# 2646207530/hamer-yolo

Measured on AMD Instinct MI355X. Metric: hands/sec (HaMeR ViT-H/16 + decoder + MANO forward; detector bypassed), higher is better.
Workload: dtype fp16; 1 GPU; BASELINE configs[1]: batch=64 synthetic 256x256 crops per GPU, HaMeR ViT-H/16 + 6-layer decoder + MANO, 16-bit MFMA (fp16 operands), crops resident in HBM; batch_per_gpu=64, global_batch=64, batches_in_flight=2, weights=seeded random-init fp32 master weights, rounded to the operand type at load, parallelism=crop-shard x1

## Files before the change

hamer_yolo_amd/csrc/attention.hip:

```cpp
#include "common.h"
#include "hamer_hip_internal.h"

namespace {

constexpr int T = 192;
constexpr int HD = 80;
constexpr int KSTR = 88;
constexpr int VSTR = 80;
constexpr int KS_BYTES = T * KSTR * 2;
constexpr int VT_BYTES = T * VSTR * 2;
constexpr int BUF_BYTES = KS_BYTES + VT_BYTES;
constexpr int NWAVE = T / 16;
constexpr int OTILE_BYTES = 16 * HD * 2;
constexpr int ATT_LDS = 2 * BUF_BYTES + NWAVE * OTILE_BYTES;
constexpr int ATT_LDS_TOME = ATT_LDS + 2 * T * 4;

template <class V4> __device__ __forceinline__ V4 lds_read_tr4(const void* p) {
  typedef __attribute__((ext_vector_type(4))) short s16x4;
  const s16x4 v = __builtin_amdgcn_ds_read_tr16_b64_v4i16((__attribute__((address_space(3))) s16x4*)p);
  return __builtin_bit_cast(V4, v);
}

__device__ __forceinline__ void glds16_hidden(const void* gsrc, void* lds_wave_base) {
  const unsigned dst = __builtin_amdgcn_readfirstlane((unsigned)(uintptr_t)(__attribute__((address_space(3))) void*)lds_wave_base);
  asm volatile("s_mov_b32 m0, %1\n\ts_nop 0\n\tglobal_load_lds_dwordx4 %0, off" :: "v"(gsrc), "s"(dst) : "memory");
}

__device__ __forceinline__ void wait_vm0() {
  __builtin_amdgcn_s_waitcnt(0x0F70);
  asm volatile("" ::: "memory");
}

constexpr int HDP = 96;
typedef __attribute__((ext_vector_type(4))) int v4i_att;

template <class TT, bool MX8 = false, bool TOME = false>
__global__ __launch_bounds__(64 * NWAVE, 3) void vit_attention_kernel(const typename TT::elem* __restrict__ qkv,
                                                                    typename TT::elem* __restrict__ out, int heads,
                                                                    int items, float scale_log2e,
                                                                    unsigned char* __restrict__ out_scales = nullptr,
                                                                    const float* __restrict__ size = nullptr, int Tn = T) {
  extern __shared__ __attribute__((aligned(16))) char smem[];
  using elem = typename TT::elem;
  using vec8 = typename TT::vec8;
  using vec4 = typename TT::vec4;

  const int tid = threadIdx.x, lane = tid & 63;
  const int wave = __builtin_amdgcn_readfirstlane(tid >> 6);
  const int C = heads * HD;
  const size_t ld = (size_t)3 * C;
  const int g = lane >> 4, li = lane & 15;
  const int Tt = TOME ? Tn : T;
  vec8 zero8;
#pragma unroll
  for (int i = 0; i < 8; ++i) zero8[i] = (elem)0.0f;
  if constexpr (TOME) {
    for (int buf = 0; buf < 2; ++buf) {
      char* Vb = smem + buf * BUF_BYTES + KS_BYTES;
      for (int c = Tt * (VSTR / 8) + tid; c < T * (VSTR / 8); c += 64 * NWAVE) *(vec8*)(Vb + c * 16) = zero8;
    }
  }

  auto issue = [&](int item, int buf, vec8 (&qf)[3], float& szl) {
    const elem* base = qkv + (size_t)(item / heads) * Tt * ld + (size_t)(item % heads) * HD;
    char* Kb = smem + buf * BUF_BYTES;
    char* Vb = Kb + KS_BYTES;
    constexpr int KCH = T * (KSTR / 8), VCH = T * (VSTR / 8);
    const int kch = Tt * (KSTR / 8), vch = Tt * (VSTR / 8);
    for (int c0 = wave * 64; c0 < KCH; c0 += 64 * NWAVE) {
      const int c = c0 + lane, ch = c % (KSTR / 8);
      int t = c / (KSTR / 8);
      if (TOME) t = t < Tt ? t : Tt - 1;
      if (!TOME || c0 < kch) glds16_hidden(base + (size_t)t * ld + C + (ch < HD / 8 ? ch : 0) * 8, Kb + c0 * 16);
    }
    for (int c0 = wave * 64; c0 < VCH; c0 += 64 * NWAVE) {
      const int c = c0 + lane, ch = c % (VSTR / 8);
      int t = c / (VSTR / 8);
      if (TOME) t = t < Tt ? t : Tt - 1;
      if (!TOME || c0 < vch) glds16_hidden(base + (size_t)t * ld + 2 * C + ch * 8, Vb + c0 * 16);
    }
    const int qr = wave * 16 + li;
    const elem* qrow = base + (size_t)(TOME ? (qr < Tt ? qr : Tt - 1) : qr) * ld;
    if constexpr (TOME) szl = (size != nullptr && tid < Tt) ? size[(size_t)(item / heads) * Tt + tid] : 1.0f;
    qf[0] = *(const vec8*)(qrow + 8 * g);
    qf[1] = *(const vec8*)(qrow + 32 + 8 * g);
    qf[2] = g < 2 ? *(const vec8*)(qrow + 64 + 8 * g) : zero8;
  };

  auto compute = [&](int item, int buf, const vec8 (&qf)[3]) {
    const elem* Ks = (const elem*)(smem + buf * BUF_BYTES);
    const elem* Vs = (const elem*)(smem + buf * BUF_BYTES + KS_BYTES);
    const int b = item / heads, h = item % heads;
    const int q = wave * 16 + li;
    if constexpr (TOME) { if (wave * 16 >= Tt) return; }
    f32x4_t st[12];
    vec8 kf[2][2][3];
    auto load_k = [&](int kb, int pair) {
#pragma unroll
      for (int j = 0; j < 2; ++j) {
        const elem* krow = Ks + ((pair * 2 + j) * 16 + li) * KSTR + 8 * g;
        kf[kb][j][0] = *(const vec8*)(krow);
        kf[kb][j][1] = *(const vec8*)(krow + 32);
        kf[kb][j][2] = g < 2 ? *(const vec8*)(krow + 64) : zero8;
      }
    };
    load_k(0, 0);
#pragma unroll
    for (int pair = 0; pair < 6; ++pair) {
      if (pair + 1 < 6) load_k((pair + 1) & 1, pair + 1);
#pragma unroll
      for (int j = 0; j < 2; ++j) {
        f32x4_t acc = f32x4_t{0.f, 0.f, 0.f, 0.f};
        acc = TT::mfma(kf[pair & 1][j][0], qf[0], acc);
        acc = TT::mfma(kf[pair & 1][j][1], qf[1], acc);
        acc = TT::mfma(kf[pair & 1][j][2], qf[2], acc);
        st[pair * 2 + j] = acc;
      }
    }
    if constexpr (TOME) {
#pragma unroll
      for (int kt = 0; kt < 12; ++kt) {
        const f32x4_t lz = *(const f32x4_t*)(smem + ATT_LDS + (buf * T + kt * 16 + 4 * g) * 4);
#pragma unroll
        for (int r = 0; r < 4; ++r) st[kt][r] = (kt * 16 + 4 * g + r < Tt) ? fmaf(st[kt][r], scale_log2e, lz[r]) : -INFINITY;
      }
    }
    float m = st[0][0];
#pragma unroll
    for (int kt = 0; kt < 12; ++kt)
#pragma unroll
      for (int r = 0; r < 4; ++r) m = fmaxf(m, st[kt][r]);
    m = fmaxf(m, __shfl_xor(m, 16, 64));
    m = fmaxf(m, __shfl_xor(m, 32, 64));
    const float mneg = TOME ? -m : -m * scale_log2e;
    float sum4[4] = {0.f, 0.f, 0.f, 0.f};
#pragma unroll
    for (int kt = 0; kt < 12; ++kt)
#pragma unroll
      for (int r = 0; r < 4; ++r) {
        const float p = __builtin_amdgcn_exp2f(TOME ? st[kt][r] + (mneg + 14.0f) : fmaf(st[kt][r], scale_log2e, mneg));
        st[kt][r] = p;
        sum4[r] += p;
      }
    float sum = (sum4[0] + sum4[1]) + (sum4[2] + sum4[3]);
    sum += __shfl_xor(sum, 16, 64);
    sum += __shfl_xor(sum, 32, 64);
    const float inv = 1.0f / sum;

    vec8 pf[6], pl[TOME ? 6 : 1];
#pragma unroll
    for (int kk = 0; kk < 6; ++kk)
#pragma unroll
      for (int r = 0; r < 4; ++r) {
        pf[kk][r] = (elem)st[2 * kk][r];
        pf[kk][4 + r] = (elem)st[2 * kk + 1][r];
        if constexpr (TOME) {
          pl[kk][r] = (elem)(st[2 * kk][r] - (float)pf[kk][r]);
          pl[kk][4 + r] = (elem)(st[2 * kk + 1][r] - (float)pf[kk][4 + r]);
        }
      }

    const elem* vblk = Vs + (4 * g + (li >> 2)) * VSTR + 4 * (li & 3);
    vec4 vlo[2][5], vhi[2][5];
    auto load_v = [&](int vb, int kk) {
#pragma unroll
      for (int dt = 0; dt < 5; ++dt) {
        vlo[vb][dt] = lds_read_tr4<vec4>(vblk + (32 * kk) * VSTR + dt * 16);
        vhi[vb][dt] = lds_read_tr4<vec4>(vblk + (32 * kk + 16) * VSTR + dt * 16);
      }
    };
    f32x4_t oacc[5];
#pragma unroll
    for (int dt = 0; dt < 5; ++dt) oacc[dt] = f32x4_t{0.f, 0.f, 0.f, 0.f};
    if constexpr (!TOME) load_v(0, 0);
#pragma unroll
    for (int kk = 0; kk < 6; ++kk) {
      if constexpr (TOME) load_v(kk & 1, kk);
      else if (kk + 1 < 6) load_v((kk + 1) & 1, kk + 1);
#pragma unroll
      for (int dt = 0; dt < 5; ++dt) {
        vec8 vf;
#pragma unroll
        for (int i = 0; i < 4; ++i) { vf[i] = vlo[kk & 1][dt][i]; vf[4 + i] = vhi[kk & 1][dt][i]; }
        oacc[dt] = TT::mfma(vf, pf[kk], oacc[dt]);
        if constexpr (TOME) oacc[dt] = TT::mfma(vf, pl[kk], oacc[dt]);
      }
    }
    if constexpr (MX8) {
      const int Mrows = (items / heads) * T;
      float am[3] = {0.f, 0.f, 0.f};
#pragma unroll
      for (int dt = 0; dt < 5; ++dt)
#pragma unroll
        for (int r = 0; r < 4; ++r) am[dt >> 1] = fmaxf(am[dt >> 1], fabsf(oacc[dt][r] * inv));
      unsigned sb[3];
      float isc[3];
#pragma unroll
      for (int bk = 0; bk < 3; ++bk) {
        float a = am[bk];
        a = fmaxf(a, __shfl_xor(a, 16, 64));
        a = fmaxf(a, __shfl_xor(a, 32, 64));
        sb[bk] = mx8_scale_byte(a);
        isc[bk] = mx8_inv_scale(sb[bk]);
      }
      char* ot8 = smem + 2 * BUF_BYTES + wave * OTILE_BYTES;
#pragma unroll
      for (int dt = 0; dt < 6; ++dt) {
        int p = 0;
        if (dt < 5) {
          const float sc = inv * isc[dt >> 1];
          p = mx8_pack4(oacc[dt][0] * sc, oacc[dt][1] * sc, oacc[dt][2] * sc, oacc[dt][3] * sc);
        }
        *(int*)(ot8 + li * HDP + dt * 16 + 4 * g) = p;
      }
      char* obase8 = (char*)out + ((size_t)b * T + wave * 16) * (heads * HDP) + h * HDP;
#pragma unroll
      for (int c0 = 0; c0 < 16 * (HDP / 16); c0 += 64) {
        const int c = c0 + lane;
        if (c < 16 * (HDP / 16)) {
          const int row = c / (HDP / 16), ch = c % (HDP / 16);
          *(v4i_att*)(obase8 + (size_t)row * (heads * HDP) + ch * 16) = *(const v4i_att*)(ot8 + row * HDP + ch * 16);
        }
      }
      if (g == 0) {
#pragma unroll
        for (int bk = 0; bk < 3; ++bk) out_scales[(size_t)(h * 3 + bk) * Mrows + (size_t)b * T + q] = (unsigned char)sb[bk];
      }
      return;
    }
    elem* ot = (elem*)(smem + 2 * BUF_BYTES + wave * OTILE_BYTES);
#pragma unroll
    for (int dt = 0; dt < 5; ++dt) {
      vec4 o;
#pragma unroll
      for (int r = 0; r < 4; ++r) o[r] = (elem)(oacc[dt][r] * inv);
      *(vec4*)(ot + li * HD + dt * 16 + 4 * g) = o;
    }
    elem* obase = out + ((size_t)b * Tt + wave * 16) * C + h * HD;
#pragma unroll
    for (int c0 = 0; c0 < 16 * (HD / 8); c0 += 64) {
      const int c = c0 + lane;
      if (c < 16 * (HD / 8)) {
        const int row = c / (HD / 8), ch = c % (HD / 8);
        if (!TOME || wave * 16 + row < Tt) *(vec8*)(obase + (size_t)row * C + ch * 8) = *(const vec8*)(ot + row * HD + ch * 8);
      }
    }
  };

  vec8 qa[3], qb[3];
  float sza = 1.0f, szb = 1.0f;
  auto publish_size = [&](int buf, float szl) {
    if constexpr (TOME) { if (tid < Tt) *(float*)(smem + ATT_LDS + (buf * T + tid) * 4) = __builtin_amdgcn_logf(szl); }
  };
  int item = xcd_remap(blockIdx.x, gridDim.x);
  if (item < items) issue(item, 0, qa, sza);
  while (item < items) {
    wait_vm0();
    publish_size(0, sza);
    __builtin_amdgcn_s_barrier();
    int nxt = item + gridDim.x;
    if (nxt < items) issue(nxt, 1, qb, szb);
    compute(item, 0, qa);
    item = nxt;
    if (item >= items) break;
    wait_vm0();
    publish_size(1, szb);
    __builtin_amdgcn_s_barrier();
    nxt = item + gridDim.x;
    if (nxt < items) issue(nxt, 0, qa, sza);
    compute(item, 1, qb);
    item = nxt;
  }
}

int att_grid_for(int items, int n_cu) {
  if (const int v = hm_option(HM_OPT_ATT_GRID)) n_cu = v;
  const int per = (items + n_cu - 1) / n_cu;
  return (items + per - 1) / per;
}

template <class TT, bool MX8 = false, bool TOME = false>
int launch_att(const void* qkv, void* out, int B, int heads, float scale, hipStream_t s, void* out_scales = nullptr,
               const float* size = nullptr, int Tn = T) {
  static HmLdsOnce lds_once;
  auto kern = vit_attention_kernel<TT, MX8, TOME>;
  constexpr int LDS = TOME ? ATT_LDS_TOME : ATT_LDS;
  if (const int rc = lds_once.ensure((const void*)kern, LDS, "hm_vit_attention: cannot raise dynamic LDS limit")) return rc;
  const int n_cu = hm_device_cu_count();
  if (n_cu <= 0) return hm_set_error(HM_ERR_HIP, "hm_vit_attention: cannot query the device");
  const int items = B * heads;
  const int grid = att_grid_for(items, n_cu);
  hipLaunchKernelGGL(kern, dim3(grid), dim3(64 * NWAVE), LDS, s, (const typename TT::elem*)qkv,
                     (typename TT::elem*)out, heads, items, scale * 1.44269504088896340736f, (unsigned char*)out_scales, size, Tn);
  return hm_check_launch("hm_vit_attention");
}

}

extern "C" int hm_attention_grid(int items, int cus) {
  if (items <= 0) return 0;
  return att_grid_for(items, cus > 0 ? cus : 256);
}

int hm_attention_tome_launch(const void* qkv, const float* size, void* out, int B, int tokens, int heads, float scale, int dtype,
                             hipStream_t s) {
  if (tokens < 1 || tokens > T) return hm_set_error(HM_ERR_ARG, "hm_tome_attention: 0 < tokens <= 192");
  if (dtype == HM_DTYPE_BF16) return launch_att<TBf16, false, true>(qkv, out, B, heads, scale, s, nullptr, size, tokens);
  if (dtype == HM_DTYPE_F16) return launch_att<TF16, false, true>(qkv, out, B, heads, scale, s, nullptr, size, tokens);
  return hm_set_error(HM_ERR_ARG, "hm_tome_attention: bad dtype");
}

extern "C" int hm_vit_attention(const void* qkv, void* out, int B, int tokens, int heads, int head_dim, float scale,
                                int dtype, void* stream_) {
  hipStream_t s = (hipStream_t)stream_;
  if (!qkv || !out || B <= 0 || heads <= 0) return hm_set_error(HM_ERR_ARG, "hm_vit_attention: bad arguments");
  if (tokens != T || head_dim != HD)
    return hm_set_error(HM_ERR_ARG, "hm_vit_attention: built for 192 tokens and head_dim 80 (ViT-H/16 on 256x192)");
  if (((uintptr_t)qkv | (uintptr_t)out) & 15) return hm_set_error(HM_ERR_ARG, "hm_vit_attention: 16-byte alignment");
  HmProfScope prof(HM_K_ATTENTION, 0, B, heads, head_dim, s);
  if (dtype == HM_DTYPE_BF16) return launch_att<TBf16>(qkv, out, B, heads, scale, s);
  if (dtype == HM_DTYPE_F16) return launch_att<TF16>(qkv, out, B, heads, scale, s);
  return hm_set_error(HM_ERR_ARG, "hm_vit_attention: bad dtype");
}

extern "C" int hm_vit_attention_mx8(const void* qkv, void* out8, void* out_scales, int B, int tokens, int heads, int head_dim,
                                    float scale, void* stream_) {
  hipStream_t s = (hipStream_t)stream_;
  if (!qkv || !out8 || !out_scales || B <= 0 || heads <= 0) return hm_set_error(HM_ERR_ARG, "hm_vit_attention_mx8: bad arguments");
  if (tokens != T || head_dim != HD)
    return hm_set_error(HM_ERR_ARG, "hm_vit_attention_mx8: built for 192 tokens and head_dim 80 (ViT-H/16 on 256x192)");
  if (((uintptr_t)qkv | (uintptr_t)out8 | (uintptr_t)out_scales) & 15) return hm_set_error(HM_ERR_ARG, "hm_vit_attention_mx8: 16-byte alignment");
  HmProfScope prof(HM_K_ATTENTION, 1, B, heads, head_dim, s);
  return launch_att<TBf16, true>(qkv, out8, B, heads, scale, s, out_scales);
}
```

Baseline: 3728 hands/s.

## Use partial vmcnt waits and unconditional Q loads in attention prefetch ring

For the non-ToMe attention path, the kernel now waits only until the previous item's K/V loads retire (vmcnt<=3), leaving the next item's output stores in flight, instead of draining all outstanding memory ops each iteration. The third Q fragment is loaded without a lane-dependent branch, and the zero masking is moved into compute. Output write-back loops are flattened into fixed-count stores without bounds checks. The intent is to cut stalls from full vmcnt drains and from divergent tails. The risk is that the vmcnt count depends on the exact instruction ordering the compiler emits, which could cause correctness hazards.

Result: no change. 3730 hands/s (median of 2 runs) (+0.1%).

```diff
diff --git a/hamer_yolo_amd/csrc/attention.hip b/hamer_yolo_amd/csrc/attention.hip
--- a/hamer_yolo_amd/csrc/attention.hip
+++ b/hamer_yolo_amd/csrc/attention.hip
@@ -21,18 +21,20 @@
   return __builtin_bit_cast(V4, v);
 }
 
-__device__ __forceinline__ void glds16_hidden(const void* gsrc, void* lds_wave_base) {
-  const unsigned dst = __builtin_amdgcn_readfirstlane((unsigned)(uintptr_t)(__attribute__((address_space(3))) void*)lds_wave_base);
+__device__ __forceinline__ void glds16_hidden(const void* gsrc, unsigned lds_wave_base) {
+  const unsigned dst = __builtin_amdgcn_readfirstlane(lds_wave_base);
   asm volatile("s_mov_b32 m0, %1\n\ts_nop 0\n\tglobal_load_lds_dwordx4 %0, off" :: "v"(gsrc), "s"(dst) : "memory");
 }
 
-__device__ __forceinline__ void wait_vm0() {
-  __builtin_amdgcn_s_waitcnt(0x0F70);
+template <int N> __device__ __forceinline__ void wait_vm() {
+  static_assert(N >= 0 && N < 16, "vmcnt immediate");
   asm volatile("" ::: "memory");
-}
-
+  __builtin_amdgcn_s_waitcnt(0x0F70 | N);
+  asm volatile("" ::: "memory");
+}
 constexpr int HDP = 96;
 typedef __attribute__((ext_vector_type(4))) int v4i_att;
+typedef __attribute__((ext_vector_type(2))) int v2i_att;
 
 template <class TT, bool MX8 = false, bool TOME = false>
 __global__ __launch_bounds__(64 * NWAVE, 3) void vit_attention_kernel(const typename TT::elem* __restrict__ qkv,
@@ -51,6 +53,8 @@
   const size_t ld = (size_t)3 * C;
   const int g = lane >> 4, li = lane & 15;
   const int Tt = TOME ? Tn : T;
+  constexpr bool RING = !TOME;
+  constexpr int N_ST = 3;
   vec8 zero8;
 #pragma unroll
   for (int i = 0; i < 8; ++i) zero8[i] = (elem)0.0f;
@@ -61,11 +65,11 @@
     }
   }
 
-  auto issue = [&](int item, int buf, vec8 (&qf)[3], float& szl) {
-    const elem* base = qkv + (size_t)(item / heads) * Tt * ld + (size_t)(item % heads) * HD;
-    char* Kb = smem + buf * BUF_BYTES;
-    char* Vb = Kb + KS_BYTES;
-    constexpr int KCH = T * (KSTR / 8), VCH = T * (VSTR / 8);
+  constexpr int KCH_ALL = T * (KSTR / 8), VCH_ALL = T * (VSTR / 8);
+  auto copy_kv = [&](const elem* base, int buf) {
+    const unsigned Kb = (unsigned)(uintptr_t)(__attribute__((address_space(3))) char*)smem + buf * BUF_BYTES;
+    const unsigned Vb = Kb + KS_BYTES;
+    constexpr int KCH = KCH_ALL, VCH = VCH_ALL;
     const int kch = Tt * (KSTR / 8), vch = Tt * (VSTR / 8);
     for (int c0 = wave * 64; c0 < KCH; c0 += 64 * NWAVE) {
       const int c = c0 + lane, ch = c % (KSTR / 8);
@@ -79,12 +83,17 @@
       if (TOME) t = t < Tt ? t : Tt - 1;
       if (!TOME || c0 < vch) glds16_hidden(base + (size_t)t * ld + 2 * C + ch * 8, Vb + c0 * 16);
     }
+  };
+  auto issue = [&](int item, int buf, vec8 (&qf)[3], float& szl) {
+    const elem* base = qkv + (size_t)(item / heads) * Tt * ld + (size_t)(item % heads) * HD;
+    copy_kv(base, buf);
     const int qr = wave * 16 + li;
     const elem* qrow = base + (size_t)(TOME ? (qr < Tt ? qr : Tt - 1) : qr) * ld;
     if constexpr (TOME) szl = (size != nullptr && tid < Tt) ? size[(size_t)(item / heads) * Tt + tid] : 1.0f;
     qf[0] = *(const vec8*)(qrow + 8 * g);
     qf[1] = *(const vec8*)(qrow + 32 + 8 * g);
-    qf[2] = g < 2 ? *(const vec8*)(qrow + 64 + 8 * g) : zero8;
+    if constexpr (RING) qf[2] = *(const vec8*)(qrow + 64 + 8 * (g & 1));
+    else qf[2] = g < 2 ? *(const vec8*)(qrow + 64 + 8 * g) : zero8;
   };
 
   auto compute = [&](int item, int buf, const vec8 (&qf)[3]) {
@@ -95,6 +104,7 @@
     if constexpr (TOME) { if (wave * 16 >= Tt) return; }
     f32x4_t st[12];
     vec8 kf[2][2][3];
+    const vec8 q2 = (!RING || g < 2) ? qf[2] : zero8;
     auto load_k = [&](int kb, int pair) {
 #pragma unroll
       for (int j = 0; j < 2; ++j) {
@@ -113,7 +123,7 @@
         f32x4_t acc = f32x4_t{0.f, 0.f, 0.f, 0.f};
         acc = TT::mfma(kf[pair & 1][j][0], qf[0], acc);
         acc = TT::mfma(kf[pair & 1][j][1], qf[1], acc);
-        acc = TT::mfma(kf[pair & 1][j][2], qf[2], acc);
+        acc = TT::mfma(kf[pair & 1][j][2], q2, acc);
         st[pair * 2 + j] = acc;
       }
     }
@@ -214,18 +224,14 @@
         *(int*)(ot8 + li * HDP + dt * 16 + 4 * g) = p;
       }
       char* obase8 = (char*)out + ((size_t)b * T + wave * 16) * (heads * HDP) + h * HDP;
-#pragma unroll
-      for (int c0 = 0; c0 < 16 * (HDP / 16); c0 += 64) {
-        const int c = c0 + lane;
-        if (c < 16 * (HDP / 16)) {
-          const int row = c / (HDP / 16), ch = c % (HDP / 16);
-          *(v4i_att*)(obase8 + (size_t)row * (heads * HDP) + ch * 16) = *(const v4i_att*)(ot8 + row * HDP + ch * 16);
-        }
-      }
-      if (g == 0) {
-#pragma unroll
-        for (int bk = 0; bk < 3; ++bk) out_scales[(size_t)(h * 3 + bk) * Mrows + (size_t)b * T + q] = (unsigned char)sb[bk];
-      }
+      {
+        const int row = lane / (HDP / 16), ch = lane % (HDP / 16);
+        *(v4i_att*)(obase8 + (size_t)row * (heads * HDP) + ch * 16) = *(const v4i_att*)(ot8 + row * HDP + ch * 16);
+        const int e = 64 * 16 + 8 * lane, row2 = e / HDP, col2 = e % HDP;
+        *(v2i_att*)(obase8 + (size_t)row2 * (heads * HDP) + col2) = *(const v2i_att*)(ot8 + row2 * HDP + col2);
+      }
+      const int bk = g < 2 ? g : 2;
+      out_scales[(size_t)(h * 3 + bk) * Mrows + (size_t)b * T + q] = (unsigned char)(g == 0 ? sb[0] : g == 1 ? sb[1] : sb[2]);
       return;
     }
     elem* ot = (elem*)(smem + 2 * BUF_BYTES + wave * OTILE_BYTES);
@@ -237,13 +243,23 @@
       *(vec4*)(ot + li * HD + dt * 16 + 4 * g) = o;
     }
     elem* obase = out + ((size_t)b * Tt + wave * 16) * C + h * HD;
-#pragma unroll
-    for (int c0 = 0; c0 < 16 * (HD / 8); c0 += 64) {
-      const int c = c0 + lane;
-      if (c < 16 * (HD / 8)) {
-        const int row = c / (HD / 8), ch = c % (HD / 8);
-        if (!TOME || wave * 16 + row < Tt) *(vec8*)(obase + (size_t)row * C + ch * 8) = *(const vec8*)(ot + row * HD + ch * 8);
-      }
+    if constexpr (TOME) {
+#pragma unroll
+      for (int c0 = 0; c0 < 16 * (HD / 8); c0 += 64) {
+        const int c = c0 + lane;
+        if (c < 16 * (HD / 8)) {
+          const int row = c / (HD / 8), ch = c % (HD / 8);
+          if (wave * 16 + row < Tt) *(vec8*)(obase + (size_t)row * C + ch * 8) = *(const vec8*)(ot + row * HD + ch * 8);
+        }
+      }
+    } else {
+#pragma unroll
+      for (int c0 = 0; c0 < 128; c0 += 64) {
+        const int c = c0 + lane, row = c / (HD / 8), ch = c % (HD / 8);
+        *(vec8*)(obase + (size_t)row * C + ch * 8) = *(const vec8*)(ot + row * HD + ch * 8);
+      }
+      const int e = 128 * 8 + 4 * lane, row = e / HD, col = e % HD;
+      *(vec4*)(obase + (size_t)row * C + col) = *(const vec4*)(ot + row * HD + col);
     }
   };
 
@@ -253,23 +269,49 @@
     if constexpr (TOME) { if (tid < Tt) *(float*)(smem + ATT_LDS + (buf * T + tid) * 4) = __builtin_amdgcn_logf(szl); }
   };
   int item = xcd_remap(blockIdx.x, gridDim.x);
-  if (item < items) issue(item, 0, qa, sza);
-  while (item < items) {
-    wait_vm0();
-    publish_size(0, sza);
+  if constexpr (!RING) {
+    if (item < items) issue(item, 0, qa, sza);
+    while (item < items) {
+      wait_vm<0>();
+      publish_size(0, sza);
+      __builtin_amdgcn_s_barrier();
+      int nxt = item + gridDim.x;
+      if (nxt < items) issue(nxt, 1, qb, szb);
+      compute(item, 0, qa);
+      item = nxt;
+      if (item >= items) break;
+      wait_vm<0>();
+      publish_size(1, szb);
+      __builtin_amdgcn_s_barrier();
+      nxt = item + gridDim.x;
+      if (nxt < items) issue(nxt, 0, qa, sza);
+      compute(item, 1, qb);
+      item = nxt;
+    }
+  } else {
+    if (item >= items) return;
+    issue(item, 0, qa, sza);
+    wait_vm<0>();
     __builtin_amdgcn_s_barrier();
     int nxt = item + gridDim.x;
     if (nxt < items) issue(nxt, 1, qb, szb);
     compute(item, 0, qa);
     item = nxt;
-    if (item >= items) break;
-    wait_vm0();
-    publish_size(1, szb);
-    __builtin_amdgcn_s_barrier();
-    nxt = item + gridDim.x;
-    if (nxt < items) issue(nxt, 0, qa, sza);
-    compute(item, 1, qb);
-    item = nxt;
+    while (item < items) {
+      wait_vm<N_ST>();
+      __builtin_amdgcn_s_barrier();
+      nxt = item + gridDim.x;
+      if (nxt < items) issue(nxt, 0, qa, sza);
+      compute(item, 1, qb);
+      item = nxt;
+      if (item >= items) break;
+      wait_vm<N_ST>();
+      __builtin_amdgcn_s_barrier();
+      nxt = item + gridDim.x;
+      if (nxt < items) issue(nxt, 1, qb, szb);
+      compute(item, 0, qa);
+      item = nxt;
+    }
   }
 }
 
```
